# jolibrain/joliGEN

Measured on AMD Instinct MI355X. Metric: train images/sec at 256x256 (DDPM UNet step), higher is better.
Workload: dtype bf16; 1 GPU; palette_model DDPM, efficient UNet unet_mha ngf64 mults[1,2,4,8] res_blocks[2,2,2,2] mid-attn 16x32, 256x256, batch 32/GPU, inpainting synthetic masks, AdamW+EMA, iter_size 1 (example_ddpm_noglasses2glasses.json + SURVEY Appendix C overrides); global_batch=32, per_gpu_batch=32, image_size=256, efficient=True, parallelism=dp1, n_ranks_seen=1

## Files before the change

joligen_amd/_lib.py:

```python
from __future__ import annotations

import ctypes as C
import os
import subprocess

_HERE = os.path.dirname(os.path.abspath(__file__))
CSRC = os.path.join(_HERE, "csrc")
LIB_PATH = os.path.join(CSRC, "libjg355.so")
SOURCES = ["attention.hip", "gemm_nt.hip", "conv_halo.hip", "conv_kxk.hip", "reflect_border.hip", "conv_p64.hip", "conv1x1.hip", "gemm_tn.hip", "wgrad_halo.hip", "wgrad_sw.hip", "wgrad_kxk.hip", "nce.hip", "segformer.hip", "vit.hip", "projected_d.hip", "effnet.hip", "norm.hip", "gn_fused.hip", "elementwise.hip", "d_aug.hip", "resize_aa.hip", "optim.hip", "capi.hip"]
HIPCC_FLAGS = ["--offload-arch=gfx950", "-O3", "-std=c++17", "-fPIC", "-shared", "-munsafe-fp-atomics", "-fno-slp-vectorize"]

FILE_FLAGS = {}

JG_OK, JG_ERR_BAD_ARG, JG_ERR_UNSUPPORTED, JG_ERR_LAUNCH = 0, -1, -2, -3
JG_F16, JG_BF16 = 0, 1
JG_ACT_NONE, JG_ACT_SILU, JG_ACT_RELU, JG_ACT_LRELU, JG_ACT_TANH = 0, 1, 2, 3, 4
JG_OUT_ATOMIC_F32, JG_OUT_STORE_F32, JG_OUT_STORE_T = 0, 1, 2

c_i32, c_i64, c_f32, c_p = C.c_int32, C.c_int64, C.c_float, C.c_void_p


class ConvArgs(C.Structure):
    _fields_ = (
        [(n, c_p) for n in ("x", "w", "y", "bias", "res")]
        + [(n, c_i32) for n in ("B", "H", "W", "Cin", "Cout", "R", "S", "pad", "stride", "Ho", "Wo")]
        + [(n, c_i64) for n in ("ldx", "ldw", "ldy", "ldres")]
        + [(n, c_i32) for n in ("nbatch", "nh")]
        + [(n, c_i64) for n in ("sxb", "sxh", "swb", "swh", "syb", "syh", "srb", "srh")]
        + [("alpha", c_f32), ("res_scale", c_f32), ("out_f32", c_i32), ("stats", c_p), ("ldstats", c_i64), ("stats_slots", c_i32), ("stats_mode", c_i32), ("gn_x", c_p), ("gn_ldx", c_i64), ("gn_ab", c_p), ("gn_act", c_i32), ("pad_mode", c_i32), ("res_mode", c_i32), ("x_mode", c_i32), ("y_mode", c_i32), ("ws", c_p), ("ws_bytes", c_i64)]
    )


class WgradArgs(C.Structure):
    _fields_ = (
        [(n, c_p) for n in ("dy", "x", "dw", "dbias")]
        + [(n, c_i32) for n in ("B", "H", "W", "Cin", "Cout", "R", "S", "pad", "stride", "Ho", "Wo")]
        + [(n, c_i32) for n in ("Cin_out", "Cout_out")]
        + [(n, c_i64) for n in ("lddy", "ldx", "lddw")]
        + [(n, c_i32) for n in ("nbatch", "nh", "splitk")]
        + [(n, c_i64) for n in ("sdyb", "sdyh", "sxb", "sxh", "sdwb", "sdwh")]
        + [("alpha", c_f32), ("out_mode", c_i32), ("dbias_scale", c_f32), ("pad_mode", c_i32), ("x_mode", c_i32)]
    )


SIGNATURES = {
    "jg_version": [],
    "jg_strerror": [c_i32],
    "jg_set_tuning": [C.c_char_p, c_i32],
    "jg_get_tuning": [C.c_char_p],
    "jg_last_kernel": [],
    "jg_conv2d_nt": [c_i32, C.POINTER(ConvArgs), c_p],
    "jg_conv1x1_gn_apply": [c_i32, C.POINTER(ConvArgs), c_p, c_p, c_i64, c_i32, c_p],
    "jg_conv1x1_gn_bwd_apply": [c_i32, C.POINTER(ConvArgs), c_p, c_i64, c_p, c_i64, c_p, c_p, c_p, c_i64, c_f32, c_p, c_i64, c_f32, c_i32, c_p],
    "jg_conv2d_wgrad_tn": [c_i32, C.POINTER(WgradArgs), c_p],
    "jg_conv2d_wgrad_tn_group": [c_i32, C.POINTER(WgradArgs), c_i32, c_p],
    "jg_gn_stats": [c_i32, c_p, c_p, c_i32, c_i32, c_i32, c_p],
    "jg_gn_coef": [c_p, c_p, c_p, c_p, c_i64, c_p, c_p, c_i32, c_i32, c_i32, c_i32, c_f32, c_p],
    "jg_gn_apply": [c_i32, c_p, c_p, c_p, c_i32, c_i32, c_i32, c_i32, c_p],
    "jg_gn_apply_add": [c_i32, c_p, c_i64, c_p, c_p, c_i64, c_p, c_i64, c_i32, c_i32, c_i32, c_i32, c_p],
    "jg_gn_bwd_reduce": [c_i32, c_p, c_p, c_p, c_p, c_i32, c_i32, c_i32, c_i32, c_p],
    "jg_subpixel_fold": [c_i32, c_p, c_p, c_i32, c_i32, c_p],
    "jg_transposed_fold": [c_i32, c_p, c_p, c_i32, c_i32, c_i32, c_i32, c_i32, c_p],
    "jg_gn_apply_pool": [c_i32, c_p, c_i64, c_p, c_p, c_i64, c_i32, c_i32, c_i32, c_i32, c_i32, c_f32, c_p],
    "jg_gn_bwd_reduce_up": [c_i32, c_p, c_i64, c_p, c_i64, c_f32, c_p, c_p, c_i32, c_i32, c_i32, c_i32, c_i32, c_p],
    "jg_gn_bwd_reduce_up_acc": [c_i32, c_p, c_i64, c_p, c_i64, c_f32, c_p, c_p, c_i32, c_i32, c_i32, c_i32, c_i32, c_p],
    "jg_gn_bwd_fused": [c_i32, c_i32, c_p, c_i64, c_p, c_i64, c_f32, c_p, c_p, c_p, c_p, c_p, c_p, c_p, c_i64, c_p, c_p, c_p, c_p, c_i64, c_i32, c_p, c_i64,
                        c_p, c_i64, c_f32, c_p, c_i64, c_f32, c_i32, c_i32, c_i32, c_i32, c_i32, c_p],
    "jg_gn_bwd_apply_fc": [c_i32, c_i32, c_p, c_i64, c_p, c_i64, c_f32, c_p, c_p, c_p, c_p, c_p, c_i64, c_p, c_p, c_p, c_p, c_i64, c_i32, c_p, c_i64,
                           c_p, c_i64, c_f32, c_p, c_i64, c_f32, c_i32, c_i32, c_i32, c_i32, c_i32, c_p],
    "jg_gn_bwd_reduce_ld_acc": [c_i32, c_p, c_i64, c_p, c_i64, c_p, c_p, c_i32, c_i32, c_i32, c_i32, c_p],
    "jg_gn_bwd_apply_up": [c_i32, c_p, c_i64, c_p, c_i64, c_f32, c_p, c_p, c_p, c_i64, c_p, c_i64, c_f32, c_p, c_i64, c_f32, c_i32, c_i32,
                           c_i32, c_i32, c_i32, c_p],
    "jg_gn_bwd_coef": [c_p, c_p, c_p, c_p, c_i64, c_p, c_p, c_p, c_p, c_p, c_i64, c_i32, c_i32, c_i32, c_i32, c_p],
    "jg_gn_bwd_coef_slots": [c_p, c_i32, c_p, c_p, c_p, c_i64, c_p, c_p, c_p, c_p, c_p, c_i64, c_i32, c_i32, c_i32, c_i32, c_p],
    "jg_gn_bwd_apply": [c_i32, c_p, c_p, c_p, c_p, c_p, c_i32, c_i32, c_i32, c_i32, c_p],
    "jg_gn_stats_ld": [c_i32, c_p, c_i64, c_p, c_i64, c_i32, c_i32, c_i32, c_p],
    "jg_gn_coef_ld": [c_p, c_i64, c_i32, c_p, c_p, c_p, c_i64, c_p, c_p, c_i32, c_i32, c_i32, c_i32, c_f32, c_p],
    "jg_gn_apply_ld": [c_i32, c_p, c_i64, c_p, c_p, c_i64, c_i32, c_i32, c_i32, c_i32, c_p],
    "jg_gn_bwd_reduce_ld": [c_i32, c_p, c_i64, c_p, c_i64, c_p, c_p, c_i32, c_i32, c_i32, c_i32, c_p],
    "jg_gn_bwd_apply_ld": [c_i32, c_p, c_i64, c_p, c_i64, c_p, c_p, c_p, c_i64, c_p, c_i64, c_f32, c_p, c_i64, c_f32,
                           c_i32, c_i32, c_i32, c_i32, c_p],
    "jg_pool2x2": [c_i32, c_p, c_p, c_i32, c_i32, c_i32, c_i32, c_f32, c_p],
    "jg_upsample2x": [c_i32, c_p, c_p, c_i32, c_i32, c_i32, c_i32, c_f32, c_p],
    "jg_pool2x2_ld": [c_i32, c_p, c_i64, c_p, c_i64, c_i32, c_i32, c_i32, c_i32, c_f32, c_p],
    "jg_upsample2x_ld": [c_i32, c_p, c_i64, c_p, c_i64, c_i32, c_i32, c_i32, c_i32, c_f32, c_p],
    "jg_copy_channels": [c_i32, c_p, c_i64, c_i64, c_p, c_i64, c_i64, c_i64, c_i32, c_p],
    "jg_axpby": [c_i32, c_p, c_f32, c_p, c_p, c_f32, c_p, c_i64, c_p],
    "jg_transpose_heads": [c_i32, c_p, c_i64, c_i64, c_i64, c_p, c_i32, c_i32, c_i32, c_i32, c_p],
    "jg_softmax_fwd": [c_i32, c_p, c_p, c_i64, c_i32, c_p],
    "jg_softmax_bwd": [c_i32, c_p, c_p, c_p, c_i64, c_i32, c_f32, c_p],
    "jg_attention_fwd": [c_i32, c_p, c_p, c_p, c_i32, c_i32, c_i32, c_i32, c_p],
    "jg_attention_bwd": [c_i32, c_p, c_p, c_p, c_p, c_p, c_p, c_i32, c_i32, c_i32, c_i32, c_p],
# ... 189 lines not shown
```

joligen_amd/csrc/capi.hip:

```cpp
#include "common.h"

extern "C" int jg_version(void) { return 100; }

extern "C" const char* jg_strerror(int code) {
  switch (code) {
    case JG_OK: return "ok";
    case JG_ERR_BAD_ARG: return "bad argument (null pointer, misaligned leading dimension or unsupported shape)";
    case JG_ERR_UNSUPPORTED: return "unsupported configuration";
    case JG_ERR_LAUNCH: return "HIP launch failed";
    default: return "unknown error";
  }
}

#include <atomic>
#include <cstdlib>
#include <cstring>
#include <mutex>

namespace {
struct TuneDef { const char* env; int dflt; };
const TuneDef kTune[JG_TUNE_COUNT] = {
    {"JG_HALO_CFG", 0}, {"JG_WGRAD_HALO_CFG", 0}, {"JG_CONV_VARIANT", 6}, {"JG_WGRAD_VARIANT", 4}, {"JG_SINKHORN_GENERIC", 0},
    {"JG_CONV1X1", 1}, {"JG_GN_REVERSE", 1}, {"JG_HALO_DBG", 0}, {"JG_PERSIST64", 1}, {"JG_HALO_PIPE", 1}, {"JG_WGRAD_PIPE", 1}, {"JG_CONV_SPLITK", 1}, {"JG_CONV_SMALL_TILE", 1}, {"JG_GN_FUSED", 1}, {"JG_GN_FUSED_CAP", 256}, {"JG_GN_FUSED_DBG", 0}, {"JG_GN_FUSED_SLEEP", 4}, {"JG_WGRAD_LDS_PAD", 0},
    {"JG_LN_BWD_CAP", 256}, {"JG_DW_BWD_CAP", 512}, {"JG_DW_BWD_PPT", 8}, {"JG_CONV_KXK", 1}, {"JG_CONV_RING", 1}, {"JG_WGRAD_DEEP", 1}, {"JG_WGRAD_SW", 0}, {"JG_DETERMINISTIC", 0}, {"JG_WGRAD_GROUP_BLOCKS", 1024}, {"JG_SGEMM_SPLIT", 0}, {"JG_WGRAD_BIG", 1}, {"JG_DW_RUN", 1}};
std::atomic<int> g_tune[JG_TUNE_COUNT];
std::once_flag g_tune_once;
void tune_init() {
  for (int i = 0; i < JG_TUNE_COUNT; ++i) {
    const char* e = getenv(kTune[i].env);
    g_tune[i].store(e ? atoi(e) : kTune[i].dflt, std::memory_order_relaxed);
  }
}
}

namespace {
thread_local const char* g_last_kernel = "";
}
void jg_note_kernel(const char* name) { g_last_kernel = name ? name : ""; }
extern "C" const char* jg_last_kernel(void) { return g_last_kernel; }

int jg_tune(int which) {
  std::call_once(g_tune_once, tune_init);
  return g_tune[which].load(std::memory_order_relaxed);
}

extern "C" int jg_set_tuning(const char* name, int value) {
  if (!name) return JG_ERR_BAD_ARG;
  std::call_once(g_tune_once, tune_init);
  for (int i = 0; i < JG_TUNE_COUNT; ++i)
    if (!strcmp(name, kTune[i].env)) {
      g_tune[i].store(value, std::memory_order_relaxed);
      return JG_OK;
    }
  return JG_ERR_BAD_ARG;
}

extern "C" int jg_get_tuning(const char* name) {
  if (!name) return -1;
  for (int i = 0; i < JG_TUNE_COUNT; ++i)
    if (!strcmp(name, kTune[i].env)) return jg_tune(i);
  return -1;
}
```

joligen_amd/csrc/common.h:

```cpp
#pragma once
#include <hip/hip_runtime.h>
#include <stdint.h>

#include "../../include/jg355.h"

typedef _Float16 f16_t;
typedef __bf16 bf16_t;
typedef _Float16 f16x8 __attribute__((ext_vector_type(8)));
typedef __bf16 bf16x8 __attribute__((ext_vector_type(8)));
typedef float f32x4 __attribute__((ext_vector_type(4)));

#define JG_WAVE 64

enum JgTune { JG_TUNE_HALO_CFG = 0, JG_TUNE_WGRAD_HALO_CFG, JG_TUNE_CONV_VARIANT, JG_TUNE_WGRAD_VARIANT, JG_TUNE_SINKHORN_GENERIC,
              JG_TUNE_CONV1X1, JG_TUNE_GN_REVERSE, JG_TUNE_HALO_DBG, JG_TUNE_PERSIST64, JG_TUNE_HALO_PIPE, JG_TUNE_WGRAD_PIPE, JG_TUNE_CONV_SPLITK, JG_TUNE_CONV_SMALL_TILE, JG_TUNE_GN_FUSED, JG_TUNE_GN_FUSED_CAP, JG_TUNE_GN_FUSED_DBG, JG_TUNE_GN_FUSED_SLEEP, JG_TUNE_WGRAD_LDS_PAD,
              JG_TUNE_LN_BWD_CAP, JG_TUNE_DW_BWD_CAP, JG_TUNE_DW_BWD_PPT, JG_TUNE_CONV_KXK, JG_TUNE_CONV_RING, JG_TUNE_WGRAD_DEEP, JG_TUNE_WGRAD_SW, JG_TUNE_DETERMINISTIC, JG_TUNE_WGRAD_GROUP_BLOCKS, JG_TUNE_SGEMM_SPLIT, JG_TUNE_WGRAD_BIG, JG_TUNE_DW_RUN, JG_TUNE_COUNT };
int jg_tune(int which);
void jg_note_kernel(const char* name);

#define JG_CHECK_LAUNCH()                          \
  do {                                             \
    if (hipGetLastError() != hipSuccess) return JG_ERR_LAUNCH; \
  } while (0)

template <typename T> __device__ __forceinline__ float to_f32(T v) { return (float)v; }
template <typename T> __device__ __forceinline__ T from_f32(float v) { return (T)v; }

template <typename T> __device__ __forceinline__ T bits_to(uint16_t b) { return __builtin_bit_cast(T, b); }
template <typename T> __device__ __forceinline__ uint16_t to_bits(T v) { return __builtin_bit_cast(uint16_t, v); }

template <typename T> __device__ __forceinline__ void unpack8(const uint4& v, float* f) {
  const uint32_t w[4] = {v.x, v.y, v.z, v.w};
#pragma unroll
  for (int i = 0; i < 4; ++i) {
    f[2 * i] = to_f32(bits_to<T>((uint16_t)(w[i] & 0xffffu)));
    f[2 * i + 1] = to_f32(bits_to<T>((uint16_t)(w[i] >> 16)));
  }
}
template <typename T> __device__ __forceinline__ uint4 pack8(const float* f) {
  uint32_t w[4];
#pragma unroll
  for (int i = 0; i < 4; ++i) {
    w[i] = (uint32_t)to_bits<T>(from_f32<T>(f[2 * i])) | ((uint32_t)to_bits<T>(from_f32<T>(f[2 * i + 1])) << 16);
  }
  return make_uint4(w[0], w[1], w[2], w[3]);
}
template <typename T> __device__ __forceinline__ uint2 pack4(float a, float b, float c, float d) {
  uint2 r;
  r.x = (uint32_t)to_bits<T>(from_f32<T>(a)) | ((uint32_t)to_bits<T>(from_f32<T>(b)) << 16);
  r.y = (uint32_t)to_bits<T>(from_f32<T>(c)) | ((uint32_t)to_bits<T>(from_f32<T>(d)) << 16);
  return r;
}
template <typename T> __device__ __forceinline__ void unpack4(const uint2& v, float* f) {
  f[0] = to_f32(bits_to<T>((uint16_t)(v.x & 0xffffu)));
  f[1] = to_f32(bits_to<T>((uint16_t)(v.x >> 16)));
  f[2] = to_f32(bits_to<T>((uint16_t)(v.y & 0xffffu)));
  f[3] = to_f32(bits_to<T>((uint16_t)(v.y >> 16)));
}

template <typename T> struct Mfma;
template <> struct Mfma<f16_t> {
  static __device__ __forceinline__ f32x4 run(const uint4& a, const uint4& b, f32x4 c) {
    return __builtin_amdgcn_mfma_f32_16x16x32_f16(__builtin_bit_cast(f16x8, a), __builtin_bit_cast(f16x8, b), c, 0, 0, 0);
  }
};
template <> struct Mfma<bf16_t> {
  static __device__ __forceinline__ f32x4 run(const uint4& a, const uint4& b, f32x4 c) {
    return __builtin_amdgcn_mfma_f32_16x16x32_bf16(__builtin_bit_cast(bf16x8, a), __builtin_bit_cast(bf16x8, b), c, 0, 0, 0);
  }
};

template <typename T> __device__ __forceinline__ uint4 ldg16(const T* ptr, bool ok) {
  uint4 v = *reinterpret_cast<const uint4*>(ptr);
  v.x = ok ? v.x : 0u;
  v.y = ok ? v.y : 0u;
  v.z = ok ? v.z : 0u;
  v.w = ok ? v.w : 0u;
  return v;
}

__device__ __forceinline__ float sigmoid_fast(float u) { return __builtin_amdgcn_rcpf(1.0f + __expf(-u)); }
__device__ __forceinline__ float silu_f(float u) { return u * sigmoid_fast(u); }
__device__ __forceinline__ float silu_grad_f(float u) {
  const float s = sigmoid_fast(u);
  return s * (1.0f + u * (1.0f - s));
}

template <int ACT> __device__ __forceinline__ float act_f(float u) {
  if (ACT == JG_ACT_SILU) return silu_f(u);
  if (ACT == JG_ACT_RELU) return fmaxf(u, 0.f);
  if (ACT == JG_ACT_LRELU) return u > 0.f ? u : 0.2f * u;
  return u;
}
template <int ACT> __device__ __forceinline__ float act_grad_f(float u) {
  if (ACT == JG_ACT_SILU) return silu_grad_f(u);
  if (ACT == JG_ACT_RELU) return u > 0.f ? 1.f : 0.f;
  if (ACT == JG_ACT_LRELU) return u > 0.f ? 1.f : 0.2f;
  return 1.f;
}
// ... 36 lines not shown
```

joligen_amd/csrc/conv_params.h:

```cpp
#pragma once
#define JG_REFLECT1(i, n) ((i) < 0 ? -(i) : ((i) >= (n) ? 2 * ((n) - 1) - (i) : (i)))
#include "common.h"

struct ConvP {
  const char* x; const char* w; char* y; const float* bias; const char* res;
  int M, N, K;
  int H, W, Cin, R, S, pad, stride, Ho, Wo;
  long ldx, ldw, ldy, ldres;
  int nh;
  long sxb, sxh, swb, swh, syb, syh, srb, srh;
  float alpha, res_scale;
  int out_f32;
  int B;
  float* stats;
  long ldstats;
  int nslots;
  int stats_mode;
  int dbg;
  const char* gx; long gldx; const float* gab; int gact;
  int y_pool;
  int x_up;
  int res_up;
  int reflect;
  float* ws; int splitk;
  const float* aab; char* ay; long lday; int aact;
  const char* bgx; long bldgx; const char* bgdy; long bldgdy; const float* bab; const float* bpqr;
  const char* badd1; long bldadd1; float bsc1; const char* badd2; long bldadd2; float bsc2; int bact;
};

__device__ __forceinline__ long jg_res_up_row(const ConvP& p, long m) {
  const int ow = (int)(m % p.Wo);
  const long t = m / p.Wo;
  const int oh = (int)(t % p.Ho);
  const long b = t / p.Ho;
  return (b * (p.Ho >> 1) + (oh >> 1)) * (p.Wo >> 1) + (ow >> 1);
}

__device__ __forceinline__ void jg_stats_flush(float* stats, long row, int n, const float* s1, const float* s2, int lane) {
#pragma unroll
  for (int q = 0; q < 4; ++q) {
    float a = s1[q], b = s2[q];
#pragma unroll
    for (int o = 1; o < 16; o <<= 1) {
      a += __shfl_xor(a, o);
      b += __shfl_xor(b, o);
    }
    if ((lane & 15) == 0) {
      atomicAdd(stats + (row + n + q) * 2, a);
      atomicAdd(stats + (row + n + q) * 2 + 1, b);
    }
  }
}

bool jg_conv_halo_try(int dtype, const ConvP& p, int nbatch, hipStream_t st);
bool jg_conv_p64_try(int dtype, const ConvP& p, int nbatch, hipStream_t st);
bool jg_conv1x1_try(int dtype, const ConvP& p, int nbatch, hipStream_t st);
bool jg_conv_kxk_try(int dtype, const ConvP& p, int nbatch, hipStream_t st);
```

joligen_amd/csrc/gemm_nt.hip:

```cpp
#include "common.h"
#include "conv_params.h"
#include "conv_epilogue.h"
#include <cstdlib>
#include <type_traits>

namespace {


__device__ __forceinline__ int swz64(int row) { return ((row >> 3) & 1) << 1; }

template <typename T, int BM, int BN, int WAVES_M, int WAVES_N>
__global__ __launch_bounds__(256) void conv_nt_kernel(ConvP p) {
  constexpr int WM = BM / WAVES_M, WN = BN / WAVES_N;
  constexpr int TM = WM / 16, TN = WN / 16;
  constexpr int A_CH = BM * 4 / 256, B_CH = BN * 4 / 256;
  static_assert(WAVES_M * WAVES_N == 4, "4 waves");
  static_assert(A_CH >= 1 && B_CH >= 1, "tile too small");

  __shared__ uint4 sm[2][(BM + BN) * 4];

  const int tid = threadIdx.x;
  const int lane = tid & 63;
  const int wave = tid >> 6;
  const int wm = wave / WAVES_N, wn = wave % WAVES_N;
// ... 392 lines not shown
  const long idx = (long)blockIdx.x * 256 + threadIdx.x;
  if (idx >= total) return;
  const int n = (int)(idx % n4) * 4;
  const long zm = idx / n4;
  const long m = zm % p.M;
  const int z = (int)(zm / p.M);
  const int zb = z / p.nh, zh = z % p.nh;
  const long slice = (long)nbatch * p.M * p.N;
  const float* src = p.ws + (long)z * p.M * p.N + m * p.N + n;
  float4 a = *reinterpret_cast<const float4*>(src);
  for (int sp = 1; sp < p.splitk; ++sp) {
    const float4 b = *reinterpret_cast<const float4*>(src + sp * slice);
    a.x += b.x; a.y += b.y; a.z += b.z; a.w += b.w;
  }
  float v[4] = {p.alpha * a.x, p.alpha * a.y, p.alpha * a.z, p.alpha * a.w};
  if (p.bias) {
#pragma unroll
    for (int q = 0; q < 4; ++q) v[q] += p.bias[n + q];
  }
  if (p.res) {
    const T* resb = (const T*)p.res + zb * p.srb + zh * p.srh;
    float rf[4];
    unpack4<T>(*reinterpret_cast<const uint2*>(resb + m * p.ldres + n), rf);
#pragma unroll
    for (int q = 0; q < 4; ++q) v[q] += p.res_scale * rf[q];
  }
  char* yb = p.y + (zb * p.syb + zh * p.syh) * (p.out_f32 ? 4 : 2);
  if (p.out_f32) *reinterpret_cast<float4*>((float*)yb + m * p.ldy + n) = make_float4(v[0], v[1], v[2], v[3]);
  else *reinterpret_cast<uint2*>((T*)yb + m * p.ldy + n) = pack4<T>(v[0], v[1], v[2], v[3]);
}

static int pick_conv_splitk(long blocks, int nk, long out_elems, long ws_bytes) {
  if (blocks >= 128 || nk < 16) return 1;
  int sk = (int)((256 + blocks - 1) / blocks);
  if (sk > nk / 4) sk = nk / 4;
  if (sk > 32) sk = 32;
  while (sk > 1 && (long)sk * out_elems * 4 > ws_bytes) --sk;
  return sk < 2 ? 1 : sk;
}

template <typename T, int BM, int BN, int BK, int WMv, int WNv>
void launch_glds(ConvP p, int nbatch, hipStream_t st, long ws_bytes = 0) {
  const long blocks = (long)((p.M + BM - 1) / BM) * ((p.N + BN - 1) / BN) * nbatch;
  p.splitk = 1;
  if (p.ws && !p.stats && !p.res_up && (p.N & 3) == 0 && jg_tune(JG_TUNE_CONV_SPLITK))
    p.splitk = pick_conv_splitk(blocks, (p.K + BK - 1) / BK, (long)nbatch * p.M * p.N, ws_bytes);
  dim3 grid(((p.M + BM - 1) / BM) * ((p.N + BN - 1) / BN), p.splitk, nbatch);
  constexpr bool has_ring = BK == 64 && BM == BN && (BM == 64 || BM == 128);
  const int ring = jg_tune(JG_TUNE_CONV_RING);
  const bool use_ring = has_ring && ring && p.splitk == 1 && (ring >= 2 || ((p.K + BK - 1) / BK >= 8 && blocks <= (BM == 64 ? 512 : 256)));
  if constexpr (has_ring) {
    if (use_ring) {
      hipLaunchKernelGGL((conv_nt_glds_kernel<T, BM, BN, BK, WMv, WNv, false, BM == 64 ? 4 : 3>), grid, dim3(256), 0, st, p);
      return;
    }
  }
  if (p.splitk > 1) hipLaunchKernelGGL((conv_nt_glds_kernel<T, BM, BN, BK, WMv, WNv, true>), grid, dim3(256), 0, st, p);
  else hipLaunchKernelGGL((conv_nt_glds_kernel<T, BM, BN, BK, WMv, WNv, false>), grid, dim3(256), 0, st, p);
  if (p.splitk > 1) {
    jg_note_kernel(BM == 64 ? "conv_nt_glds_kernel<64,64,64,2,2>+splitK" : BN == 32 ? "conv_nt_glds_kernel<256,32,64,4,1>+splitK"
                   : BN == 64 ? "conv_nt_glds_kernel<256,64,64,4,1>+splitK" : "conv_nt_glds_kernel<128,128,64,2,2>+splitK");
    const long total = (long)nbatch * p.M * (p.N >> 2);
    hipLaunchKernelGGL((splitk_finalize_kernel<T>), dim3((unsigned)((total + 255) / 256)), dim3(256), 0, st, p, nbatch);
  }
}

template <typename T>
int launch_conv(const ConvP& p, int nbatch, hipStream_t st, long ws_bytes) {
  const int variant = jg_tune(JG_TUNE_CONV_VARIANT);
  if (p.stats && variant < 2) return JG_ERR_UNSUPPORTED;
  if (variant >= 6 && !p.reflect && jg_conv1x1_try(sizeof(T) == 2 && std::is_same<T, f16_t>::value ? JG_F16 : JG_BF16, p, nbatch, st)) {
    JG_CHECK_LAUNCH();
    return JG_OK;
  }
  if (variant >= 6 && jg_conv_p64_try(sizeof(T) == 2 && std::is_same<T, f16_t>::value ? JG_F16 : JG_BF16, p, nbatch, st)) {
    JG_CHECK_LAUNCH();
    return JG_OK;
  }
  if (variant >= 6 && jg_conv_halo_try(sizeof(T) == 2 && std::is_same<T, f16_t>::value ? JG_F16 : JG_BF16, p, nbatch, st)) {
    JG_CHECK_LAUNCH();
    return JG_OK;
  }
  if (variant >= 6 && jg_conv_kxk_try(sizeof(T) == 2 && std::is_same<T, f16_t>::value ? JG_F16 : JG_BF16, p, nbatch, st)) {
    JG_CHECK_LAUNCH();
    return JG_OK;
  }
  if (p.reflect || p.x_up || p.y_pool) return JG_ERR_UNSUPPORTED;
  if (variant >= 2) {
    const long b128 = (long)((p.M + 127) / 128) * ((p.N + 127) / 128) * nbatch;
    const long b256 = (long)((p.M + 255) / 256) * ((p.N + 63) / 64) * nbatch;
    const bool can_split = p.ws && !p.stats && !p.res_up && (p.K + 63) / 64 >= 16 && jg_tune(JG_TUNE_CONV_SPLITK);
    const bool alt_ok = (variant == 3 || variant >= 6) && jg_tune(JG_TUNE_CONV_SMALL_TILE) && !(p.stats && p.stats_mode == 1);
    const long b64 = (long)((p.M + 63) / 64) * ((p.N + 63) / 64) * nbatch;
    const bool fill64 = jg_tune(JG_TUNE_CONV_SMALL_TILE) >= 1 && jg_tune(JG_TUNE_CONV_SMALL_TILE) != 2 && b64 >= 256;
    const bool small = alt_ok && (p.N <= 64 ? b256 : b128) < 160 && (!can_split || fill64);
    if (small) {
      jg_note_kernel("conv_nt_glds_kernel<64,64,64,2,2>");
      launch_glds<T, 64, 64, 64, 2, 2>(p, nbatch, st, ws_bytes);
    } else if (p.N <= 32 && alt_ok) {
      jg_note_kernel("conv_nt_glds_kernel<256,32,64,4,1>");
      launch_glds<T, 256, 32, 64, 4, 1>(p, nbatch, st, ws_bytes);
    } else if (p.N <= 64) {
      if (variant == 3 || variant >= 6) launch_glds<T, 256, 64, 64, 4, 1>(p, nbatch, st, ws_bytes);
      else launch_glds<T, 256, 64, 32, 4, 1>(p, nbatch, st);
    } else {
      if (variant == 2) launch_glds<T, 128, 128, 32, 2, 2>(p, nbatch, st);
      else if (variant == 3 || variant >= 6) launch_glds<T, 128, 128, 64, 2, 2>(p, nbatch, st, ws_bytes);
      else if (variant == 4) launch_glds<T, 256, 128, 32, 2, 2>(p, nbatch, st);
      else launch_glds<T, 256, 128, 64, 2, 2>(p, nbatch, st);
    }
    JG_CHECK_LAUNCH();
    return JG_OK;
  }
  if (p.N <= 64) {
    constexpr int BM = 256, BN = 64;
    dim3 grid(((p.M + BM - 1) / BM) * ((p.N + BN - 1) / BN), 1, nbatch);
    hipLaunchKernelGGL((conv_nt_kernel<T, BM, BN, 4, 1>), grid, dim3(256), 0, st, p);
  } else {
    constexpr int BM = 128, BN = 128;
    dim3 grid(((p.M + BM - 1) / BM) * ((p.N + BN - 1) / BN), 1, nbatch);
    hipLaunchKernelGGL((conv_nt_kernel<T, BM, BN, 2, 2>), grid, dim3(256), 0, st, p);
  }
  JG_CHECK_LAUNCH();
  return JG_OK;
}

}

static int conv_args_to_params(const jg_conv_args* a, ConvP& p);

extern "C" int jg_conv2d_nt(int dtype, const jg_conv_args* a, jg_stream_t stream) {
  jg_note_kernel("");
  ConvP p;
  const int rc = conv_args_to_params(a, p);
  if (rc != JG_OK) return rc;
  if (p.stats && jg_tune(JG_TUNE_DETERMINISTIC) != 0) {
    if (p.stats_mode != 0) return JG_ERR_UNSUPPORTED;
    float* st = p.stats;
    p.stats = nullptr;
    int r2;
    JG_DISPATCH_DTYPE(dtype, r2 = launch_conv<T>(p, a->nbatch, (hipStream_t)stream, a->ws ? (long)a->ws_bytes : 0););
    if (r2 != JG_OK) return r2;
    return jg_gn_stats_ld(dtype, a->y, a->ldy, st, (int64_t)p.nslots * p.ldstats, a->B, a->Ho * a->Wo, a->Cout, stream);
  }
  JG_DISPATCH_DTYPE(dtype, return launch_conv<T>(p, a->nbatch, (hipStream_t)stream, a->ws ? (long)a->ws_bytes : 0););
}

extern "C" int jg_conv1x1_gn_apply(int dtype, const jg_conv_args* a, const float* ab, void* y_norm, int64_t ldyn, int act, jg_stream_t stream) {
  jg_note_kernel("");
  if (!ab || !y_norm || !a || ldyn < a->Cin || (ldyn % 8)) return JG_ERR_BAD_ARG;
  ConvP p;
  const int rc = conv_args_to_params(a, p);
  if (rc != JG_OK) return rc;
  if (((long)a->Ho * a->Wo) % 16 || a->nbatch != 1) return JG_ERR_UNSUPPORTED;
  p.aab = ab; p.ay = (char*)y_norm; p.lday = ldyn; p.aact = act;
  if (!jg_conv1x1_try(dtype, p, a->nbatch, (hipStream_t)stream)) return JG_ERR_UNSUPPORTED;
  JG_CHECK_LAUNCH();
  return JG_OK;
}

extern "C" int jg_conv1x1_gn_bwd_apply(int dtype, const jg_conv_args* a, const void* gn_x, int64_t ldgx, const void* gn_dy, int64_t ldgdy,
                                       const float* ab, const float* pqr, const void* add1, int64_t ldadd1, float scale1, const void* add2,
                                       int64_t ldadd2, float scale2, int act, jg_stream_t stream) {
  jg_note_kernel("");
  if (!a || !gn_x || !gn_dy || !ab || !pqr || ldgx < a->Cout || ldgdy < a->Cout || (ldgx % 8) || (ldgdy % 8)) return JG_ERR_BAD_ARG;
  if ((add1 && (ldadd1 < a->Cout || ldadd1 % 8)) || (add2 && (ldadd2 < a->Cout || ldadd2 % 8)) || a->res || a->bias) return JG_ERR_BAD_ARG;
// ... 54 lines not shown
```

joligen_amd/csrc/gemm_tn.hip:

```cpp
#include "common.h"
#include "wgrad_params.h"
#include <vector>
#include <cstdlib>

namespace {


__device__ __forceinline__ int swz128(int row) { return (row >> 1) & 7; }

__device__ __forceinline__ void transpose4x8(const uint4* ra, uint2* out) {
  const uint32_t w[4][4] = {{ra[0].x, ra[0].y, ra[0].z, ra[0].w},
                            {ra[1].x, ra[1].y, ra[1].z, ra[1].w},
                            {ra[2].x, ra[2].y, ra[2].z, ra[2].w},
                            {ra[3].x, ra[3].y, ra[3].z, ra[3].w}};
#pragma unroll
  for (int d = 0; d < 4; ++d) {
    out[2 * d].x = (w[0][d] & 0xffffu) | (w[1][d] << 16);
    out[2 * d].y = (w[2][d] & 0xffffu) | (w[3][d] << 16);
    out[2 * d + 1].x = (w[0][d] >> 16) | (w[1][d] & 0xffff0000u);
    out[2 * d + 1].y = (w[2][d] >> 16) | (w[3][d] & 0xffff0000u);
  }
}

template <typename T>
// ... 819 lines not shown
  const int variant = jg_tune(JG_TUNE_WGRAD_VARIANT);
  if (variant < 2) return JG_ERR_UNSUPPORTED;
  std::vector<WgP> ps((size_t)n);
  std::vector<char> special((size_t)n, 0);
  for (int i = 0; i < n; ++i) {
    const int rc = make_wgp(a + i, ps[i]);
    if (rc != JG_OK) return rc;
    if (a[i].nbatch != 1 || a[i].out_mode != JG_OUT_ATOMIC_F32 || ps[i].reflect || ps[i].x_up) return JG_ERR_UNSUPPORTED;
    special[i] = variant >= 4 && (a[i].R > 1 || a[i].S > 1) &&
                 (jg_wgrad_halo_try(dtype, ps[i], 1, (hipStream_t)stream, true) || jg_wgrad_kxk_try(dtype, ps[i], 1, (hipStream_t)stream, true));
  }
  for (int i = 0; i < n; ++i)
    if (special[i] && !jg_wgrad_halo_try(dtype, ps[i], 1, (hipStream_t)stream)) jg_wgrad_kxk_try(dtype, ps[i], 1, (hipStream_t)stream);
  const int group_blocks = jg_tune(JG_TUNE_WGRAD_GROUP_BLOCKS);
  const size_t gpad = (size_t)jg_tune(JG_TUNE_WGRAD_LDS_PAD);
  for (int wavesm = 1; wavesm <= 3; ++wavesm) {
    WgGroup g;
    g.n = 0;
    g.start[0] = 0;
    auto flush = [&]() -> int {
      if (!g.n) return JG_OK;
      if (group_blocks > 0) {
        long total = 0;
        for (int i = 0; i < g.n; ++i) total += (long)g.tiles[i] * ((g.p[i].Mpix + 63) / 64);
        const long len = std::max<long>(4, (total + group_blocks - 1) / group_blocks);
        for (int i = 0; i < g.n; ++i) {
          const long ks = (g.p[i].Mpix + 63) / 64;
          g.p[i].splitk = (int)std::max<long>(1, std::min<long>(g.p[i].splitk, (ks + len - 1) / len));
          g.start[i + 1] = g.start[i] + g.tiles[i] * g.p[i].splitk;
        }
      }
      const dim3 grid(g.start[g.n]);
      const int deep = jg_tune(JG_TUNE_WGRAD_DEEP);
      if (wavesm == 3) {
        if (jg_tune(JG_TUNE_WGRAD_BIG) == 2) { JG_DISPATCH_DTYPE(dtype, hipLaunchKernelGGL((wgrad_tn_big_group_kernel<T, false>), grid, dim3(512), 0, (hipStream_t)stream, g);); }
        else { JG_DISPATCH_DTYPE(dtype, hipLaunchKernelGGL((wgrad_tn_big_group_kernel<T, true>), grid, dim3(512), 0, (hipStream_t)stream, g);); }
      } else if (wavesm == 1) {
        if (deep & 1) { JG_DISPATCH_DTYPE(dtype, hipLaunchKernelGGL((wgrad_tn_tr_group_kernel<T, 1, true>), grid, dim3(256), gpad, (hipStream_t)stream, g);); }
        else { JG_DISPATCH_DTYPE(dtype, hipLaunchKernelGGL((wgrad_tn_tr_group_kernel<T, 1>), grid, dim3(256), gpad, (hipStream_t)stream, g);); }
      } else {
        if (deep & 2) { JG_DISPATCH_DTYPE(dtype, hipLaunchKernelGGL((wgrad_tn_tr_group_kernel<T, 2, true>), grid, dim3(256), gpad, (hipStream_t)stream, g);); }
        else { JG_DISPATCH_DTYPE(dtype, hipLaunchKernelGGL((wgrad_tn_tr_group_kernel<T, 2>), grid, dim3(256), gpad, (hipStream_t)stream, g);); }
      }
      g.n = 0;
      return JG_OK;
    };
    for (int i = 0; i < n; ++i) {
      const WgP& p = ps[i];
      if (special[i] || (wg_big_ok(p) ? 3 : p.Cout <= 64 ? 1 : 2) != wavesm) continue;
      const int tiles = wavesm == 3 ? ((p.Cout + 255) / 256) * ((p.Ktot + 255) / 256) : ((p.Cout + 64 * wavesm - 1) / (64 * wavesm)) * ((p.Ktot + 127) / 128);
      g.p[g.n] = p;
      g.tiles[g.n] = tiles;
      g.start[g.n + 1] = g.start[g.n] + tiles * p.splitk;
      if (++g.n == GROUP_MAX) {
        const int rc2 = flush();
        if (rc2 != JG_OK) return rc2;
      }
    }
    const int rc3 = flush();
    if (rc3 != JG_OK) return rc3;
  }
  JG_CHECK_LAUNCH();
  return JG_OK;
}

extern "C" int jg_conv2d_wgrad_tn(int dtype, const jg_wgrad_args* a, jg_stream_t stream) {
  jg_note_kernel("");
  WgP p;
  {
    const int rc = make_wgp(a, p);
    if (rc != JG_OK) return rc;
  }
  const int variant = jg_tune(JG_TUNE_WGRAD_VARIANT);
  if (variant >= 4 && (jg_wgrad_halo_try(dtype, p, a->nbatch, (hipStream_t)stream) || jg_wgrad_kxk_try(dtype, p, a->nbatch, (hipStream_t)stream))) {
    JG_CHECK_LAUNCH();
    return JG_OK;
  }
  if (p.reflect || p.x_up) return JG_ERR_UNSUPPORTED;
  if (variant >= 2 && wg_big_ok(p)) {
    const int tiles = ((p.Cout + 255) / 256) * ((p.Ktot + 255) / 256);
    dim3 grid(tiles, 1, a->nbatch * p.splitk);
    jg_note_kernel("wgrad_tn_big_kernel");
    const int bigmode = jg_tune(JG_TUNE_WGRAD_BIG);
    if (bigmode == 11) { JG_DISPATCH_DTYPE(dtype, hipLaunchKernelGGL((wgrad_tn_big_kernel<T, true, 1>), grid, dim3(512), 0, (hipStream_t)stream, p);); }
    else if (bigmode == 12) { JG_DISPATCH_DTYPE(dtype, hipLaunchKernelGGL((wgrad_tn_big_kernel<T, true, 2>), grid, dim3(512), 0, (hipStream_t)stream, p);); }
    else if (bigmode == 14) { JG_DISPATCH_DTYPE(dtype, hipLaunchKernelGGL((wgrad_tn_big_kernel<T, true, 4>), grid, dim3(512), 0, (hipStream_t)stream, p);); }
    else if (bigmode == 13) { JG_DISPATCH_DTYPE(dtype, hipLaunchKernelGGL((wgrad_tn_big_kernel<T, true, 3>), grid, dim3(512), 0, (hipStream_t)stream, p);); }
    else if (bigmode == 2) { JG_DISPATCH_DTYPE(dtype, hipLaunchKernelGGL((wgrad_tn_big_kernel<T, false>), grid, dim3(512), 0, (hipStream_t)stream, p);); }
    else { JG_DISPATCH_DTYPE(dtype, hipLaunchKernelGGL((wgrad_tn_big_kernel<T, true>), grid, dim3(512), 0, (hipStream_t)stream, p);); }
    JG_CHECK_LAUNCH();
    return JG_OK;
  }
  const int tilesN = (p.Ktot + 127) / 128;
  if (variant == 1) {
    dim3 grid(((p.Cout + 127) / 128) * tilesN, 1, a->nbatch * p.splitk);
    JG_DISPATCH_DTYPE(dtype, hipLaunchKernelGGL((wgrad_tn_kernel<T>), grid, dim3(256), 0, (hipStream_t)stream, p););
  } else if (p.Cout <= 64 && variant != 3) {
    dim3 grid(tilesN, 1, a->nbatch * p.splitk);
    if (jg_tune(JG_TUNE_WGRAD_DEEP) & 1) { JG_DISPATCH_DTYPE(dtype, hipLaunchKernelGGL((wgrad_tn_tr_kernel<T, 1, true>), grid, dim3(256), 0, (hipStream_t)stream, p);); }
    else { JG_DISPATCH_DTYPE(dtype, hipLaunchKernelGGL((wgrad_tn_tr_kernel<T, 1>), grid, dim3(256), 0, (hipStream_t)stream, p);); }
  } else {
    dim3 grid(((p.Cout + 127) / 128) * tilesN, 1, a->nbatch * p.splitk);
    if (jg_tune(JG_TUNE_WGRAD_DEEP) & 2) { JG_DISPATCH_DTYPE(dtype, hipLaunchKernelGGL((wgrad_tn_tr_kernel<T, 2, true>), grid, dim3(256), 0, (hipStream_t)stream, p);); }
    else { JG_DISPATCH_DTYPE(dtype, hipLaunchKernelGGL((wgrad_tn_tr_kernel<T, 2>), grid, dim3(256), 0, (hipStream_t)stream, p);); }
  }
  JG_CHECK_LAUNCH();
  return JG_OK;
}
```

Before: 644.9 images/sec.

## Add pipelined 256x256 MFMA kernel for 1x1 convolutions with async LDS loads

Adds a new 1x1 convolution kernel that uses 256x256 tiles, 8 waves, and direct global-to-LDS loads with triple-buffered A and double-buffered B. This overlaps loads with MFMA compute and applies XCD-aware tile remapping. By default it is tried after the kxk path, for large 1x1 convs whose N-tile utilisation is high enough. It also puts unused wgrad ablation variants behind a compile flag to cut build size. Risks are one-workgroup-per-CU occupancy, and correctness of the fused epilogue and stats.

```diff
diff --git a/joligen_amd/_lib.py b/joligen_amd/_lib.py
--- a/joligen_amd/_lib.py
+++ b/joligen_amd/_lib.py
@@ -7,7 +7,7 @@
 _HERE = os.path.dirname(os.path.abspath(__file__))
 CSRC = os.path.join(_HERE, "csrc")
 LIB_PATH = os.path.join(CSRC, "libjg355.so")
-SOURCES = ["attention.hip", "gemm_nt.hip", "conv_halo.hip", "conv_kxk.hip", "reflect_border.hip", "conv_p64.hip", "conv1x1.hip", "gemm_tn.hip", "wgrad_halo.hip", "wgrad_sw.hip", "wgrad_kxk.hip", "nce.hip", "segformer.hip", "vit.hip", "projected_d.hip", "effnet.hip", "norm.hip", "gn_fused.hip", "elementwise.hip", "d_aug.hip", "resize_aa.hip", "optim.hip", "capi.hip"]
+SOURCES = ["attention.hip", "gemm_nt.hip", "conv_halo.hip", "conv_kxk.hip", "reflect_border.hip", "conv_p64.hip", "conv1x1.hip", "conv1x1_pipe.hip", "gemm_tn.hip", "wgrad_halo.hip", "wgrad_sw.hip", "wgrad_kxk.hip", "nce.hip", "segformer.hip", "vit.hip", "projected_d.hip", "effnet.hip", "norm.hip", "gn_fused.hip", "elementwise.hip", "d_aug.hip", "resize_aa.hip", "optim.hip", "capi.hip"]
 HIPCC_FLAGS = ["--offload-arch=gfx950", "-O3", "-std=c++17", "-fPIC", "-shared", "-munsafe-fp-atomics", "-fno-slp-vectorize"]
 
 FILE_FLAGS = {}
diff --git a/joligen_amd/csrc/capi.hip b/joligen_amd/csrc/capi.hip
--- a/joligen_amd/csrc/capi.hip
+++ b/joligen_amd/csrc/capi.hip
@@ -22,7 +22,7 @@
 const TuneDef kTune[JG_TUNE_COUNT] = {
     {"JG_HALO_CFG", 0}, {"JG_WGRAD_HALO_CFG", 0}, {"JG_CONV_VARIANT", 6}, {"JG_WGRAD_VARIANT", 4}, {"JG_SINKHORN_GENERIC", 0},
     {"JG_CONV1X1", 1}, {"JG_GN_REVERSE", 1}, {"JG_HALO_DBG", 0}, {"JG_PERSIST64", 1}, {"JG_HALO_PIPE", 1}, {"JG_WGRAD_PIPE", 1}, {"JG_CONV_SPLITK", 1}, {"JG_CONV_SMALL_TILE", 1}, {"JG_GN_FUSED", 1}, {"JG_GN_FUSED_CAP", 256}, {"JG_GN_FUSED_DBG", 0}, {"JG_GN_FUSED_SLEEP", 4}, {"JG_WGRAD_LDS_PAD", 0},
-    {"JG_LN_BWD_CAP", 256}, {"JG_DW_BWD_CAP", 512}, {"JG_DW_BWD_PPT", 8}, {"JG_CONV_KXK", 1}, {"JG_CONV_RING", 1}, {"JG_WGRAD_DEEP", 1}, {"JG_WGRAD_SW", 0}, {"JG_DETERMINISTIC", 0}, {"JG_WGRAD_GROUP_BLOCKS", 1024}, {"JG_SGEMM_SPLIT", 0}, {"JG_WGRAD_BIG", 1}, {"JG_DW_RUN", 1}};
+    {"JG_LN_BWD_CAP", 256}, {"JG_DW_BWD_CAP", 512}, {"JG_DW_BWD_PPT", 8}, {"JG_CONV_KXK", 1}, {"JG_CONV_RING", 1}, {"JG_WGRAD_DEEP", 1}, {"JG_WGRAD_SW", 0}, {"JG_DETERMINISTIC", 0}, {"JG_WGRAD_GROUP_BLOCKS", 1024}, {"JG_SGEMM_SPLIT", 0}, {"JG_WGRAD_BIG", 1}, {"JG_DW_RUN", 1}, {"JG_CONV1X1_PIPE", 1}};
 std::atomic<int> g_tune[JG_TUNE_COUNT];
 std::once_flag g_tune_once;
 void tune_init() {
diff --git a/joligen_amd/csrc/common.h b/joligen_amd/csrc/common.h
--- a/joligen_amd/csrc/common.h
+++ b/joligen_amd/csrc/common.h
@@ -14,7 +14,7 @@
 
 enum JgTune { JG_TUNE_HALO_CFG = 0, JG_TUNE_WGRAD_HALO_CFG, JG_TUNE_CONV_VARIANT, JG_TUNE_WGRAD_VARIANT, JG_TUNE_SINKHORN_GENERIC,
               JG_TUNE_CONV1X1, JG_TUNE_GN_REVERSE, JG_TUNE_HALO_DBG, JG_TUNE_PERSIST64, JG_TUNE_HALO_PIPE, JG_TUNE_WGRAD_PIPE, JG_TUNE_CONV_SPLITK, JG_TUNE_CONV_SMALL_TILE, JG_TUNE_GN_FUSED, JG_TUNE_GN_FUSED_CAP, JG_TUNE_GN_FUSED_DBG, JG_TUNE_GN_FUSED_SLEEP, JG_TUNE_WGRAD_LDS_PAD,
-              JG_TUNE_LN_BWD_CAP, JG_TUNE_DW_BWD_CAP, JG_TUNE_DW_BWD_PPT, JG_TUNE_CONV_KXK, JG_TUNE_CONV_RING, JG_TUNE_WGRAD_DEEP, JG_TUNE_WGRAD_SW, JG_TUNE_DETERMINISTIC, JG_TUNE_WGRAD_GROUP_BLOCKS, JG_TUNE_SGEMM_SPLIT, JG_TUNE_WGRAD_BIG, JG_TUNE_DW_RUN, JG_TUNE_COUNT };
+              JG_TUNE_LN_BWD_CAP, JG_TUNE_DW_BWD_CAP, JG_TUNE_DW_BWD_PPT, JG_TUNE_CONV_KXK, JG_TUNE_CONV_RING, JG_TUNE_WGRAD_DEEP, JG_TUNE_WGRAD_SW, JG_TUNE_DETERMINISTIC, JG_TUNE_WGRAD_GROUP_BLOCKS, JG_TUNE_SGEMM_SPLIT, JG_TUNE_WGRAD_BIG, JG_TUNE_DW_RUN, JG_TUNE_CONV1X1_PIPE, JG_TUNE_COUNT };
 int jg_tune(int which);
 void jg_note_kernel(const char* name);
 
diff --git a/joligen_amd/csrc/conv1x1_pipe.hip b/joligen_amd/csrc/conv1x1_pipe.hip
--- /dev/null
+++ b/joligen_amd/csrc/conv1x1_pipe.hip
@@ -0,0 +1,193 @@
+#include "conv_params.h"
+#include "conv_epilogue.h"
+#include "mfma_pipe.h"
+#include <type_traits>
+
+namespace {
+
+__device__ uint4 jg_c1p_zero_page = {0u, 0u, 0u, 0u};
+
+__device__ __forceinline__ void glds16_c1p(const void* gsrc, unsigned lds_dst) {
+  unsigned keep;
+  asm volatile("s_mov_b32 %0, m0\n\ts_mov_b32 m0, %2\n\ts_nop 0\n\tglobal_load_lds_dwordx4 %1, off\n\ts_mov_b32 m0, %0"
+               : "=&s"(keep) : "v"(gsrc), "s"(lds_dst) : "memory");
+}
+
+constexpr int C1P_BM = 256, C1P_BN = 256, C1P_NT = 512;
+
+template <typename T>
+__global__ __launch_bounds__(C1P_NT, 1) void conv1x1_pipe_kernel(ConvP p) {
+  constexpr int BM = C1P_BM, BN = C1P_BN, NT = C1P_NT, NWAVES = NT / 64, WAVES_N = 4;
+  constexpr int NA = 3, NB = 2;
+  constexpr int A_BUF = BM * 8, B_BUF = BN * 8;
+  constexpr int A_ROUNDS = A_BUF / NT, B_ROUNDS = B_BUF / NT;
+  constexpr int TM = 8, TN = 4, WN = 64;
+  static_assert(NWAVES == 2 * WAVES_N && BN == WAVES_N * WN && BM == 2 * TM * 16, "2 x 4 waves of 128 px x 64 ch");
+
+  __shared__ uint4 sm[NA * A_BUF + NB * B_BUF];
+
+  const int tid = threadIdx.x;
+  const int lane = tid & 63;
+  const int wave = __builtin_amdgcn_readfirstlane(tid >> 6);
+  const int wm = wave / WAVES_N, wn = wave % WAVES_N;
+
+  int id;
+  {
+    const int nwg = gridDim.x, q = nwg >> 3, r8 = nwg & 7, xcd = blockIdx.x & 7, idx = blockIdx.x >> 3;
+    id = (xcd < r8 ? xcd * (q + 1) : r8 * (q + 1) + (xcd - r8) * q) + idx;
+  }
+  const int tilesN = (p.N + BN - 1) / BN;
+  const int n0 = (id % tilesN) * BN;
+  const int mt = id / tilesN;
+  const int m0 = mt * BM;
+
+  const T* __restrict__ x = (const T*)p.x;
+  const T* __restrict__ w = (const T*)p.w;
+  const T* zp = reinterpret_cast<const T*>(&jg_c1p_zero_page);
+  typedef __attribute__((address_space(3))) char* lds_cptr;
+  const unsigned lds0 = (unsigned)(size_t)(lds_cptr)(char*)&sm[0];
+
+  int aoff[A_ROUNDS], boff[B_ROUNDS];
+#pragma unroll
+  for (int rd = 0; rd < A_ROUNDS; ++rd) {
+    const int row = (tid >> 3) + rd * (NT / 8);
+    const int kc = (tid & 7) ^ ((row >> 1) & 7);
+    aoff[rd] = (int)((long)(m0 + row) * p.ldx) + kc * 8;
+  }
+#pragma unroll
+  for (int rd = 0; rd < B_ROUNDS; ++rd) {
+    const int row = (tid >> 3) + rd * (NT / 8);
+    const int kc = (tid & 7) ^ ((row >> 1) & 7);
+    const int n = n0 + row;
+    boff[rd] = (n < p.N) ? (int)((long)n * p.ldw) + kc * 8 : -1;
+  }
+  auto issue_a = [&](int slot, int k) {
+#pragma unroll
+    for (int rd = 0; rd < A_ROUNDS; ++rd) glds16_c1p(x + aoff[rd] + k * 64, lds0 + (slot * A_BUF + rd * NT + wave * 64) * 16);
+  };
+  auto issue_b = [&](int slot, int k) {
+#pragma unroll
+    for (int rd = 0; rd < B_ROUNDS; ++rd)
+      glds16_c1p(boff[rd] >= 0 ? w + boff[rd] + k * 64 : zp, lds0 + (NA * A_BUF + slot * B_BUF + rd * NT + wave * 64) * 16);
+  };
+
+  f32x4 acc[TN][TM];
+#pragma unroll
+  for (int j = 0; j < TN; ++j)
+#pragma unroll
+    for (int i = 0; i < TM; ++i) acc[j][i] = (f32x4){0.f, 0.f, 0.f, 0.f};
+
+  const int l15 = lane & 15, lk = lane >> 4;
+  const unsigned afrag = (wm * (TM * 16) + l15) * 128 + ((lk ^ (l15 >> 1)) << 4);
+  const unsigned bfrag = (wn * WN + l15) * 128 + ((lk ^ (l15 >> 1)) << 4);
+
+  const int nk = p.Cin >> 6;
+  float bias_pre[8];
+
+  issue_a(0, 0);
+  if (nk > 1) issue_a(1, 1);
+  issue_b(0, 0);
+  asm volatile("s_waitcnt vmcnt(0)" ::: "memory");
+  __builtin_amdgcn_s_barrier();
+
+  u32x4 faP[8], faQ[8], fb[5];
+  jg_rd4<0, 2048, 4096, 6144>(faP[0], faP[1], faP[2], faP[3], lds0 + afrag);
+  jg_rd4<8192, 10240, 12288, 14336>(faP[4], faP[5], faP[6], faP[7], lds0 + afrag);
+
+  int aslot = 0, bslot = 0;
+  auto kstep = [&](auto lastc, int k) {
+    constexpr bool LAST = decltype(lastc)::value;
+    int anext = aslot + 1;
+    if (anext == NA) anext = 0;
+    const unsigned ab = lds0 + aslot * (A_BUF * 16), nb = lds0 + anext * (A_BUF * 16);
+    const unsigned bb = lds0 + (NA * A_BUF + bslot * B_BUF) * 16;
+    const unsigned b0 = bb + bfrag, b1 = bb + (bfrag ^ 64);
+    const unsigned a1 = ab + (afrag ^ 64), an = nb + afrag;
+    jg_rd4<0, 2048, 4096, 6144>(fb[0], fb[1], fb[2], fb[3], b0);
+    if constexpr (!LAST) {
+      issue_b(bslot ^ 1, k + 1);
+      if (k + 2 < nk) {
+        int a2 = anext + 1;
+        if (a2 == NA) a2 = 0;
+        issue_a(a2, k + 2);
+      }
+    } else {
+      jg_epilogue_bias(p, lane, n0 + wn * WN, bias_pre);
+    }
+    jg_g8r4<T, 3, 0, 2048, 4096, 6144>(acc[0], fb[0], faP, faQ[0], faQ[1], faQ[2], faQ[3], a1);
+    jg_g8r4<T, 6, 8192, 10240, 12288, 14336>(acc[1], fb[1], faP, faQ[4], faQ[5], faQ[6], faQ[7], a1);
+    jg_g8r2<T, 9, 0, 2048>(acc[2], fb[2], faP, fb[0], fb[1], b1);
+    jg_g8r2<T, 10, 4096, 6144>(acc[3], fb[3], faP, fb[2], fb[4], b1);
+    if constexpr (!LAST) {
+      jg_g8r4<T, 3, 0, 2048, 4096, 6144>(acc[0], fb[0], faQ, faP[0], faP[1], faP[2], faP[3], an);
+      jg_g8r4<T, 6, 8192, 10240, 12288, 14336>(acc[1], fb[1], faQ, faP[4], faP[5], faP[6], faP[7], an);
+      jg_g8r0<T, 9>(acc[2], fb[2], faQ);
+      jg_g8r0<T, 8>(acc[3], fb[4], faQ);
+    } else {
+      jg_g8r0<T, 3>(acc[0], fb[0], faQ);
+      jg_g8r0<T, 2>(acc[1], fb[1], faQ);
+      jg_g8r0<T, 1>(acc[2], fb[2], faQ);
+      jg_g8r0<T, 0>(acc[3], fb[4], faQ);
+    }
+    asm volatile("s_waitcnt vmcnt(0)" ::: "memory");
+    __builtin_amdgcn_s_barrier();
+    aslot = anext;
+    bslot ^= 1;
+  };
+  for (int k = 0; k + 1 < nk; ++k) kstep(std::false_type{}, k);
+  kstep(std::true_type{}, nk - 1);
+  asm volatile("s_waitcnt lgkmcnt(0)\n\ts_nop 15\n\ts_nop 15" ::: "memory");
+
+  static_assert(sizeof(sm) >= NWAVES * 16384 + BN * 8, "epilogue scratch");
+  char* smc = reinterpret_cast<char*>(&sm[0]);
+  float* sred = reinterpret_cast<float*>(smc + NWAVES * 16384);
+  if (p.stats) {
+    for (int i = tid; i < BN * 2; i += NT) sred[i] = 0.f;
+    __syncthreads();
+  }
+  const long mrow0 = (long)m0 + wm * (TM * 16);
+  const int hw = p.Ho * p.Wo;
+  const int b = p.stats ? m0 / hw : 0;
+  jg_epilogue_lds<T, TM, false>(
+      p, acc, smc + wave * 16384, lane, n0 + wn * WN, b,
+      [&](int lp) -> long { return mrow0 + lp; },
+      [&](int, long m) -> long { return m; },
+      [&](int, int, int) -> long { return 0L; },
+      [&](int nch, const float* s1, const float* s2) {
+#pragma unroll
+        for (int q = 0; q < 8; ++q) {
+          atomicAdd(&sred[(nch - n0 + q) * 2], s1[q]);
+          atomicAdd(&sred[(nch - n0 + q) * 2 + 1], s2[q]);
+        }
+      },
+      bias_pre);
+  if (p.stats) {
+    __syncthreads();
+    float* dst = p.stats + (((long)b * p.nslots + mt % p.nslots) * p.ldstats + n0) * 2;
+    const int live = (p.N - n0 < BN ? p.N - n0 : BN) * 2;
+    for (int i = tid; i < live; i += NT) atomicAdd(dst + i, sred[i]);
+  }
+}
+
+}
+
+bool jg_conv1x1_pipe_try(int dtype, const ConvP& p, int nbatch, hipStream_t st) {
+  const int mode = jg_tune(JG_TUNE_CONV1X1_PIPE);
+  if (mode == 0 || (dtype != JG_F16 && dtype != JG_BF16)) return false;
+  if (nbatch != 1 || p.R != 1 || p.S != 1 || p.pad != 0 || p.stride != 1 || p.H != p.Ho || p.W != p.Wo) return false;
+  if (p.out_f32 || p.reflect || p.x_up || p.y_pool || p.res_up || p.splitk > 1) return false;
+  if (p.Cin < 64 || p.Cin % 64 || p.N % 64 || p.M < C1P_BM || p.M % C1P_BM) return false;
+  if (p.ldx % 8 || p.ldw % 8 || p.ldy % 8 || (p.res && p.ldres % 8)) return false;
+  if (p.stats && (p.stats_mode != 0 || ((long)p.Ho * p.Wo) % C1P_BM)) return false;
+  if ((long)p.M * p.ldx >= (1L << 31) || (long)p.N * p.ldw >= (1L << 31)) return false;
+  const int tilesN = (p.N + C1P_BN - 1) / C1P_BN;
+  const long tiles = (long)(p.M / C1P_BM) * tilesN;
+  if (tiles >= (1L << 31)) return false;
+  if (mode == 1) {
+    if (tiles < 256 || 4 * p.N < 3 * tilesN * C1P_BN) return false;
+  }
+  jg_note_kernel("conv1x1_pipe_kernel<256x256,8 waves>");
+  if (dtype == JG_F16) hipLaunchKernelGGL((conv1x1_pipe_kernel<f16_t>), dim3((unsigned)tiles), dim3(C1P_NT), 0, st, p);
+  else hipLaunchKernelGGL((conv1x1_pipe_kernel<bf16_t>), dim3((unsigned)tiles), dim3(C1P_NT), 0, st, p);
+  return true;
+}
diff --git a/joligen_amd/csrc/conv_params.h b/joligen_amd/csrc/conv_params.h
--- a/joligen_amd/csrc/conv_params.h
+++ b/joligen_amd/csrc/conv_params.h
@@ -55,4 +55,5 @@
 bool jg_conv_halo_try(int dtype, const ConvP& p, int nbatch, hipStream_t st);
 bool jg_conv_p64_try(int dtype, const ConvP& p, int nbatch, hipStream_t st);
 bool jg_conv1x1_try(int dtype, const ConvP& p, int nbatch, hipStream_t st);
+bool jg_conv1x1_pipe_try(int dtype, const ConvP& p, int nbatch, hipStream_t st);
 bool jg_conv_kxk_try(int dtype, const ConvP& p, int nbatch, hipStream_t st);
diff --git a/joligen_amd/csrc/gemm_nt.hip b/joligen_amd/csrc/gemm_nt.hip
--- a/joligen_amd/csrc/gemm_nt.hip
+++ b/joligen_amd/csrc/gemm_nt.hip
@@ -498,6 +498,10 @@
     return JG_OK;
   }
   if (variant >= 6 && jg_conv_kxk_try(sizeof(T) == 2 && std::is_same<T, f16_t>::value ? JG_F16 : JG_BF16, p, nbatch, st)) {
+    JG_CHECK_LAUNCH();
+    return JG_OK;
+  }
+  if (variant >= 6 && jg_conv1x1_pipe_try(sizeof(T) == 2 && std::is_same<T, f16_t>::value ? JG_F16 : JG_BF16, p, nbatch, st)) {
     JG_CHECK_LAUNCH();
     return JG_OK;
   }
diff --git a/joligen_amd/csrc/gemm_tn.hip b/joligen_amd/csrc/gemm_tn.hip
--- a/joligen_amd/csrc/gemm_tn.hip
+++ b/joligen_amd/csrc/gemm_tn.hip
@@ -925,11 +925,14 @@
     dim3 grid(tiles, 1, a->nbatch * p.splitk);
     jg_note_kernel("wgrad_tn_big_kernel");
     const int bigmode = jg_tune(JG_TUNE_WGRAD_BIG);
+#ifdef JG_ABLATIONS
     if (bigmode == 11) { JG_DISPATCH_DTYPE(dtype, hipLaunchKernelGGL((wgrad_tn_big_kernel<T, true, 1>), grid, dim3(512), 0, (hipStream_t)stream, p);); }
     else if (bigmode == 12) { JG_DISPATCH_DTYPE(dtype, hipLaunchKernelGGL((wgrad_tn_big_kernel<T, true, 2>), grid, dim3(512), 0, (hipStream_t)stream, p);); }
     else if (bigmode == 14) { JG_DISPATCH_DTYPE(dtype, hipLaunchKernelGGL((wgrad_tn_big_kernel<T, true, 4>), grid, dim3(512), 0, (hipStream_t)stream, p);); }
     else if (bigmode == 13) { JG_DISPATCH_DTYPE(dtype, hipLaunchKernelGGL((wgrad_tn_big_kernel<T, true, 3>), grid, dim3(512), 0, (hipStream_t)stream, p);); }
-    else if (bigmode == 2) { JG_DISPATCH_DTYPE(dtype, hipLaunchKernelGGL((wgrad_tn_big_kernel<T, false>), grid, dim3(512), 0, (hipStream_t)stream, p);); }
+    else
+#endif
+    if (bigmode == 2) { JG_DISPATCH_DTYPE(dtype, hipLaunchKernelGGL((wgrad_tn_big_kernel<T, false>), grid, dim3(512), 0, (hipStream_t)stream, p);); }
     else { JG_DISPATCH_DTYPE(dtype, hipLaunchKernelGGL((wgrad_tn_big_kernel<T, true>), grid, dim3(512), 0, (hipStream_t)stream, p);); }
     JG_CHECK_LAUNCH();
     return JG_OK;
```

New measurement: 644.8 images/sec. No clear change (-0.0%).
